# noirmist/Pytorch_Pose_Proposal_Network

Measured on AMD Instinct MI355X. Metric: images/sec (384x384, DRN-D-22) at 1/2/4/8 MI355X, higher is better.
Workload: dtype bf16

## Files before the change

pytorch_pose_proposal_network_amd/csrc/stem012.hip:

```cpp
#include <hip/hip_bf16.h>

#include <cstdlib>
#include <type_traits>
#include <utility>

#include "common.h"

#ifndef PPN_S012_SKIP
#define PPN_S012_SKIP 0
#endif


namespace {

typedef __attribute__((ext_vector_type(4))) float f32x4;
typedef __attribute__((ext_vector_type(8))) __bf16 bf16x8;
typedef __attribute__((ext_vector_type(8))) _Float16 f16x8;
typedef __attribute__((ext_vector_type(4))) __bf16 bf16x4;
typedef __attribute__((ext_vector_type(2))) unsigned u32x2;
typedef __attribute__((ext_vector_type(4))) unsigned u32x4;

constexpr int SW2 = 48;
constexpr int BAND2 = 16;
constexpr int NS = 7;
constexpr int W1 = NS * 16;
constexpr int W0 = W1 + 8;
#ifdef PPN_S012_OLD_L1
constexpr int W1P = W1;
#define PPN_S012_PQ(g) (g)
#define PPN_S012_LO(g) (2 * ((g) & 1))
constexpr int kHiPlanes = 1;
#else
constexpr int W1P = W1 + 1;
#define PPN_S012_PQ(g) ((((g) & 1) << 1) | ((g) >> 1))
#define PPN_S012_LO(g) ((g) & 1)
constexpr int kHiPlanes = 2;
#endif
constexpr int WI = W1 + 8;
constexpr int R0 = 6, R1 = 5, RI = 10;
constexpr int RAWS = 368;
constexpr int LDS_IN = RI * WI * 8, LDS_L0 = R0 * W0 * 32, LDS_L1 = R1 * 4 * W1P * 8, LDS_RAW = RI * RAWS, LDS_LUT = 3 * 256 * 2;
constexpr int LDS_CST = 4 * 32 * 4;
constexpr int LDS_BYTES = LDS_IN + LDS_L0 + LDS_L1 + LDS_RAW + LDS_LUT + LDS_CST;

struct Stem012Args {
    const void* src;
    const float *w0, *s0, *b0;
    const float *w1, *s1, *b1;
    const float *w2, *s2, *b2;
    const float *s3, *b3;
    void* out_raw;
    void* out_act;
    int B, H, W, Ho, Wo, src_is_u8;
    int raw_s2;
    float mean[3], stdv[3];
    int nstrips, nbands;
};

template <typename F, int... I>
__device__ __forceinline__ void sfor_impl(F&& f, std::integer_sequence<int, I...>) {
    (f(std::integral_constant<int, I>{}), ...);
}
template <int N, typename F>
__device__ __forceinline__ void sfor(F&& f) {
    sfor_impl(f, std::make_integer_sequence<int, N>{});
}

template <int OFF>
__device__ __forceinline__ u32x2 lds_read64(unsigned addr) {
    u32x2 v;
    asm volatile("ds_read_b64 %0, %1 offset:%2" : "=v"(v) : "v"(addr), "n"(OFF));
    return v;
}

__device__ __forceinline__ f32x4 mfma16(bf16x8 a, bf16x8 b, f32x4 c, int, int, int) { return __builtin_amdgcn_mfma_f32_16x16x32_bf16(a, b, c, 0, 0, 0); }
__device__ __forceinline__ f32x4 mfma16(f16x8 a, f16x8 b, f32x4 c, int, int, int) { return __builtin_amdgcn_mfma_f32_16x16x32_f16(a, b, c, 0, 0, 0); }

template <typename H>
__device__ __forceinline__ H to_store(float v) {
    if constexpr (sizeof(H) == 2 && !__is_same(H, __bf16)) return (H)fminf(v, 65504.f);
    else return (H)v;
}

template <typename H>
__device__ __forceinline__ u32x2 bn_relu_pack(const f32x4& acc, const float (&sc)[4], const float (&sh)[4], bool inside) {
    typedef __attribute__((ext_vector_type(4))) H hx4;
    hx4 o;
#pragma unroll
    for (int r = 0; r < 4; ++r) {
        const float t = acc[r] * sc[r] + sh[r];
        o[r] = to_store<H>(t > 0.f ? t : 0.f);
    }
    u32x2 p = __builtin_bit_cast(u32x2, o);
    p.x = inside ? p.x : 0u;
    p.y = inside ? p.y : 0u;
    return p;
}

template <bool U8, typename H, typename HO = H>
__global__ void __launch_bounds__(256, 2) stem012_kernel(Stem012Args a) {
    typedef __attribute__((ext_vector_type(8))) H hx8;
    typedef __attribute__((ext_vector_type(4))) H hx4;
    typedef __attribute__((ext_vector_type(4))) HO hox4;
    constexpr bool kExactIn = U8 && std::is_same<H, _Float16>::value;
    extern __shared__ __attribute__((aligned(16))) char smem[];
    char* in_p = smem;
    char* l0_p = smem + LDS_IN;
    char* l1_p = smem + LDS_IN + LDS_L0;
    char* raw_p = smem + LDS_IN + LDS_L0 + LDS_L1;
    unsigned short* lut_p = reinterpret_cast<unsigned short*>(smem + LDS_IN + LDS_L0 + LDS_L1 + LDS_RAW);
    const int tid = threadIdx.x, lane = tid & 63;
    const int wave = __builtin_amdgcn_readfirstlane(tid >> 6);
    const int ch = lane & 15, g = lane >> 4, col = lane & 15;

    hx8 wa0[7];
    hx8 wa1[5];
    hx8 wa2[2][5];
    {
        float* wl = reinterpret_cast<float*>(smem);
        constexpr int N0 = 16 * 147, N1 = 16 * 144, N2 = 32 * 144;
        static_assert((N0 + N1 + N2) * 4 <= LDS_IN + LDS_L0 + LDS_L1, "weight staging must fit below the raw rows / LUT");
        for (int i = tid; i < N0; i += 256) wl[i] = a.w0[i];
        for (int i = tid; i < N1; i += 256) wl[N0 + i] = a.w1[i];
        for (int i = tid; i < N2; i += 256) wl[N0 + N1 + i] = a.w2[i];
        __syncthreads();
        const float* wc = wl + ch * 3 * 49;
#pragma unroll
        for (int dy = 0; dy < 7; ++dy)
#pragma unroll
            for (int hf = 0; hf < 2; ++hf) {
                const int dx = 2 * g + hf;
                const bool ok = dx < 7;
                const int dxc = ok ? dx : 6;
                float w3[3];
#pragma unroll
                for (int c = 0; c < 3; ++c) w3[c] = wc[(c * 7 + dy) * 7 + dxc];
                if constexpr (kExactIn) {
                    float v = 0.f;
#pragma unroll
                    for (int c = 0; c < 3; ++c) {
                        wa0[dy][4 * hf + c] = (H)(ok ? w3[c] / a.stdv[c] : 0.f);
                        v += w3[c] * ((128.f - a.mean[c]) / a.stdv[c]);
                    }
                    wa0[dy][4 * hf + 3] = (H)(ok ? v : 0.f);
                } else {
#pragma unroll
                    for (int c = 0; c < 3; ++c) wa0[dy][4 * hf + c] = (H)(ok ? w3[c] : 0.f);
                    wa0[dy][4 * hf + 3] = (H)0.f;
                }
            }
        const float* wd = wl + N0 + ch * 16 * 9;
#pragma unroll
        for (int kk = 0; kk < 5; ++kk) {
            const int tap = 2 * kk + (g >> 1), tapc = tap < 9 ? tap : 8;
#pragma unroll
            for (int i = 0; i < 8; ++i) {
                const float v = wd[((g & 1) * 8 + i) * 9 + tapc];
                wa1[kk][i] = (H)(tap < 9 ? v : 0.f);
            }
        }
#pragma unroll
        for (int ct = 0; ct < 2; ++ct) {
            const float* we = wl + N0 + N1 + (ct * 16 + ch) * 16 * 9;
#pragma unroll
            for (int kk = 0; kk < 5; ++kk) {
                const int tap = 2 * kk + (g >> 1), tapc = tap < 9 ? tap : 8;
#pragma unroll
                for (int i = 0; i < 8; ++i) {
                    const float v = we[((g & 1) * 8 + i) * 9 + tapc];
                    wa2[ct][kk][i] = (H)(tap < 9 ? v : 0.f);
                }
            }
        }
    }
    float sc0[4], sh0[4], sc1[4], sh1[4];
#pragma unroll
    for (int r = 0; r < 4; ++r) {
        sc0[r] = a.s0[4 * g + r]; sh0[r] = a.b0[4 * g + r];
        sc1[r] = a.s1[4 * g + r]; sh1[r] = a.b1[4 * g + r];
    }
    float* cst_p = reinterpret_cast<float*>(smem + LDS_IN + LDS_L0 + LDS_L1 + LDS_RAW + LDS_LUT);
    if (tid < 128) {
        const int c = tid & 31, which = tid >> 5;
        float v;
        if (which == 0) v = a.s2[c];
        else if (which == 1) v = a.b2[c];
        else if (which == 2) v = a.s3 ? a.s3[c] : 1.f;
        else v = a.b3 ? a.b3[c] : 0.f;
        cst_p[tid] = v;
    }
    if constexpr (U8 && !kExactIn) {
        for (int i = tid; i < 3 * 256; i += 256) {
            const int c = i >> 8;
            const H v = (H)(((float)(i & 255) - a.mean[c]) / a.stdv[c]);
            lut_p[i] = __builtin_bit_cast(unsigned short, v);
        }
    }
    int tdy[5], tdx[5];
#pragma unroll
    for (int kk = 0; kk < 5; ++kk) {
        const int tap = 2 * kk + (g >> 1), t = tap < 9 ? tap : 0;
        tdy[kk] = t / 3; tdx[kk] = t - (t / 3) * 3;
    }
    const unsigned smem_base = (unsigned)(size_t)(__attribute__((address_space(3))) char*)smem;

    const int units = a.B * a.nbands * a.nstrips;
    for (int unit = blockIdx.x; unit < units; unit += gridDim.x) {
        int u = unit;
        const int strip = u % a.nstrips; u /= a.nstrips;
        const int band = u % a.nbands;
        const int b = u / a.nbands;
        const int C2 = strip * SW2, R2 = band * BAND2;
        const int R2e = min(R2 + BAND2, a.Ho);
        const int x0b = 2 * C2 - 2;
        const int x1b = 2 * C2 - 1;
        const int xib = 2 * C2 - 5;

        const int xs = xib < 0 ? 0 : xib;
        const int nb_row = (min(xib + WI, a.W) - xs) * 3;
        auto request_input = [&](int yi0, int nrows) {
            if constexpr (U8 && !(PPN_S012_SKIP & 16)) {
                const unsigned char* base = static_cast<const unsigned char*>(a.src);
                for (int q = wave; q < nrows * 2; q += 4) {
                    const int r = q >> 1, half = q & 1;
                    const int gy = yi0 + r;
                    if (gy < 0 || gy >= a.H) continue;
                    const size_t S = (((size_t)b * a.H + gy) * a.W + xs) * 3;
                    const size_t A = S & ~(size_t)3;
                    const int k = half * 64 + lane;
                    if (k < RAWS / 4 && A + 4 * (size_t)k < S + nb_row)
                        __builtin_amdgcn_global_load_lds((const void __attribute__((address_space(1)))*)(base + A + 4 * (size_t)k),
                                                         (void __attribute__((address_space(3)))*)(raw_p + r * RAWS + half * 256),
                                                         4, 0, 0);
                }
            }
        };
        auto convert_input = [&](int yi0, int nrows) {
            if (PPN_S012_SKIP & 1) return;
            if (tid >= 2 * WI) return;
            const int prow = tid >= WI ? 1 : 0, px = tid - prow * WI;
            const int gx = xib + px;
            const bool colok = gx >= 0 && gx < a.W;
            if constexpr (U8) {
                const unsigned base = smem_base + (unsigned)(LDS_IN + LDS_L0 + LDS_L1) + prow * RAWS + (colok ? (gx - xs) * 3 : 0);
                const unsigned sh0 = (((unsigned)b * a.H + (unsigned)(yi0 + prow)) * a.W + xs) * 3u;
                const unsigned dsh = 2u * a.W * 3u;
                unsigned v[RI / 2][3];
#pragma unroll
                for (int k = 0; k < RI / 2; ++k) {
                    const unsigned ad = base + 2 * k * RAWS + ((sh0 + k * dsh) & 3u);
                    asm volatile("ds_read_u8 %0, %1" : "=v"(v[k][0]) : "v"(ad));
                    asm volatile("ds_read_u8 %0, %1 offset:1" : "=v"(v[k][1]) : "v"(ad));
                    asm volatile("ds_read_u8 %0, %1 offset:2" : "=v"(v[k][2]) : "v"(ad));
                }
#define PPN_S012_WAIT15(v)                                                                                                   \
    asm volatile("s_waitcnt lgkmcnt(0)"                                                                                     \
                 : "+v"(v[0][0]), "+v"(v[0][1]), "+v"(v[0][2]), "+v"(v[1][0]), "+v"(v[1][1]), "+v"(v[1][2]), "+v"(v[2][0]),   \
                   "+v"(v[2][1]), "+v"(v[2][2]), "+v"(v[3][0]), "+v"(v[3][1]), "+v"(v[3][2]), "+v"(v[4][0]), "+v"(v[4][1]),   \
                   "+v"(v[4][2])::"memory")
                static_assert(RI / 2 == 5, "PPN_S012_WAIT15 names 5 x 3 values");
                PPN_S012_WAIT15(v);
                if constexpr (!kExactIn) {
                    const unsigned lb = smem_base + (unsigned)(LDS_IN + LDS_L0 + LDS_L1 + LDS_RAW);
#pragma unroll
                    for (int k = 0; k < RI / 2; ++k)
#pragma unroll
                        for (int c = 0; c < 3; ++c) {
                            const unsigned ad = lb + 512 * c + 2 * v[k][c];
                            asm volatile("ds_read_u16 %0, %1" : "=v"(v[k][c]) : "v"(ad));
                        }
                    PPN_S012_WAIT15(v);
                }
#pragma unroll
                for (int k = 0; k < RI / 2; ++k) {
                    const int py = prow + 2 * k;
                    if (py >= nrows) break;
                    const int gy = yi0 + py;
                    u32x2 o = {0u, 0u};
                    if (colok && gy >= 0 && gy < a.H) {
                        if constexpr (kExactIn) {
                            hx4 t;
#pragma unroll
                            for (int c = 0; c < 3; ++c) t[c] = (H)(float)((int)v[k][c] - 128);
                            t[3] = (H)1.f;
                            o = __builtin_bit_cast(u32x2, t);
                        } else {
                            o.x = v[k][0] | (v[k][1] << 16);
                            o.y = v[k][2];
                        }
                    }
                    *reinterpret_cast<u32x2*>(in_p + ((size_t)py * WI + px) * 8) = o;
                }
            } else {
#pragma unroll
                for (int k = 0; k < RI / 2; ++k) {
                    const int py = prow + 2 * k;
                    if (py >= nrows) break;
                    const int gy = yi0 + py;
                    u32x2 o = {0u, 0u};
                    if (colok && gy >= 0 && gy < a.H) {
                        const float* sp = static_cast<const float*>(a.src) + ((size_t)b * 3 * a.H + gy) * a.W + gx;
                        const size_t plane = (size_t)a.H * a.W;
                        hx4 t;
                        t[0] = (H)sp[0]; t[1] = (H)sp[plane]; t[2] = (H)sp[2 * plane]; t[3] = (H)0.f;
                        o = __builtin_bit_cast(u32x2, t);
                    }
                    *reinterpret_cast<u32x2*>(in_p + ((size_t)py * WI + px) * 8) = o;
                }
            }
        };
        auto input_landed = [&]() {
            asm volatile("s_waitcnt vmcnt(0) lgkmcnt(0)\n\ts_barrier" ::: "memory");
        };
        auto layer0 = [&](int y, int nrows) {
            if (PPN_S012_SKIP & 2) return;
            if (wave >= nrows) return;
            const int gy = y + wave;
            const bool rowok = gy >= 0 && gy < a.H;
            const unsigned rd = smem_base + (unsigned)((wave * WI + col + 2 * g) * 8);
            char* wr = l0_p + ((size_t)(((gy + 2 * R0) % R0) * 4 + g) * W0 + col) * 8;
            u32x2 lo[2][7], hi[2][7];
            auto fetch = [&](auto sgc, auto setc) {
                constexpr int sg = decltype(sgc)::value, st = decltype(setc)::value;
                sfor<7>([&](auto dyc) {
                    constexpr int dy = decltype(dyc)::value;
                    lo[st][dy] = lds_read64<dy * WI * 8 + sg * 128>(rd);
                    hi[st][dy] = lds_read64<dy * WI * 8 + sg * 128 + 8>(rd);
                });
            };
            fetch(std::integral_constant<int, 0>{}, std::integral_constant<int, 0>{});
            sfor<NS>([&](auto sgc) {
                constexpr int sg = decltype(sgc)::value, cur = sg & 1;
                if constexpr (sg + 1 < NS) {
                    fetch(std::integral_constant<int, sg + 1>{}, std::integral_constant<int, cur ^ 1>{});
                    asm volatile("s_waitcnt lgkmcnt(14)" ::: "memory");
                } else {
                    asm volatile("s_waitcnt lgkmcnt(0)" ::: "memory");
                }
                __builtin_amdgcn_sched_barrier(0);
                f32x4 acc = {0.f, 0.f, 0.f, 0.f};
#pragma unroll
                for (int dy = 0; dy < 7; ++dy) {
                    const u32x4 xb = {lo[cur][dy].x, lo[cur][dy].y, hi[cur][dy].x, hi[cur][dy].y};
                    acc = mfma16(wa0[dy], __builtin_bit_cast(hx8, xb), acc, 0, 0, 0);
                }
                const int gx = x0b + sg * 16 + col;
                *reinterpret_cast<u32x2*>(wr + sg * 128) = bn_relu_pack<H>(acc, sc0, sh0, rowok && gx >= 0 && gx < a.W);
            });
        };
        auto layer1 = [&](int y, int nrows) {
            if (PPN_S012_SKIP & 4) return;
            if (wave >= nrows) return;
            const int gy = y + wave;
            const bool rowok = gy >= 0 && gy < a.H;
            const int s0 = (gy - 1 + 2 * R0) % R0;
            unsigned rd[5];
#pragma unroll
            for (int kk = 0; kk < 5; ++kk) {
                int s = s0 + tdy[kk];
                s = s >= R0 ? s - R0 : s;
                rd[kk] = smem_base + (unsigned)(LDS_IN + ((s * 4 + 2 * (g & 1)) * W0 + col + tdx[kk]) * 8);
            }
            char* wr = l1_p + ((size_t)(((gy + 2 * R1) % R1) * 4 + PPN_S012_PQ(g)) * W1P + col) * 8;
            u32x2 lo[2][5], hi[2][5];
            auto fetch = [&](auto sgc, auto setc) {
                constexpr int sg = decltype(sgc)::value, st = decltype(setc)::value;
#pragma unroll
                for (int kk = 0; kk < 5; ++kk) {
                    lo[st][kk] = lds_read64<sg * 128>(rd[kk]);
                    hi[st][kk] = lds_read64<sg * 128 + W0 * 8>(rd[kk]);
#ifdef PPN_S012_DUP_L1
                    lo[st][kk] = lds_read64<sg * 128>(rd[kk]);
#endif
                }
            };
            fetch(std::integral_constant<int, 0>{}, std::integral_constant<int, 0>{});
            sfor<NS>([&](auto sgc) {
                constexpr int sg = decltype(sgc)::value, cur = sg & 1;
                if constexpr (sg + 1 < NS) {
                    fetch(std::integral_constant<int, sg + 1>{}, std::integral_constant<int, cur ^ 1>{});
#ifdef PPN_S012_DUP_L1
                    asm volatile("s_waitcnt lgkmcnt(15)" ::: "memory");
#else
                    asm volatile("s_waitcnt lgkmcnt(10)" ::: "memory");
#endif
                } else {
                    asm volatile("s_waitcnt lgkmcnt(0)" ::: "memory");
                }
                __builtin_amdgcn_sched_barrier(0);
                f32x4 acc = {0.f, 0.f, 0.f, 0.f};
#pragma unroll
                for (int kk = 0; kk < 5; ++kk) {
                    const u32x4 xb = {lo[cur][kk].x, lo[cur][kk].y, hi[cur][kk].x, hi[cur][kk].y};
                    acc = mfma16(wa1[kk], __builtin_bit_cast(hx8, xb), acc, 0, 0, 0);
                }
                const int gx = x1b + sg * 16 + col;
                *reinterpret_cast<u32x2*>(wr + sg * 128) = bn_relu_pack<H>(acc, sc1, sh1, rowok && gx >= 0 && gx < a.W);
            });
        };
        auto layer2 = [&](int oy0, int nrows) {
            if (PPN_S012_SKIP & 8) return;
            const int ry = wave >> 1;
            if (ry >= nrows) return;
            const int oy = oy0 + ry;
            const int s0 = (2 * oy - 1 + 2 * R1) % R1;
            const int sg0 = (wave & 1) * 2, nsg = (wave & 1) ? 1 : 2;
            unsigned rd[5];
#pragma unroll
            for (int kk = 0; kk < 5; ++kk) {
                int s = s0 + tdy[kk];
                s = s >= R1 ? s - R1 : s;
                rd[kk] = smem_base + (unsigned)(LDS_IN + LDS_L0 + ((s * 4 + PPN_S012_LO(g)) * W1P + 2 * (sg0 * 16 + col) + tdx[kk]) * 8);
            }
            for (int sg = 0; sg < nsg; ++sg) {
                const int ox = C2 + (sg0 + sg) * 16 + col;
                u32x2 lo[5], hi[5];
#pragma unroll
                for (int kk = 0; kk < 5; ++kk) {
                    lo[kk] = lds_read64<0>(rd[kk] + sg * 256);
                    hi[kk] = lds_read64<kHiPlanes * W1P * 8>(rd[kk] + sg * 256);
                }
                asm volatile("s_waitcnt lgkmcnt(0)" ::: "memory");
                __builtin_amdgcn_sched_barrier(0);
                f32x4 acc[2] = {{0.f, 0.f, 0.f, 0.f}, {0.f, 0.f, 0.f, 0.f}};
#pragma unroll
                for (int kk = 0; kk < 5; ++kk) {
                    const u32x4 xw = {lo[kk].x, lo[kk].y, hi[kk].x, hi[kk].y};
                    const hx8 xb = __builtin_bit_cast(hx8, xw);
#pragma unroll
                    for (int ct = 0; ct < 2; ++ct)
                        acc[ct] = mfma16(wa2[ct][kk], xb, acc[ct], 0, 0, 0);
                }
                if constexpr ((PPN_S012_SKIP & 32) != 0) {
                    asm volatile("" ::"v"(acc[0]), "v"(acc[1]));
                    continue;
                }
                if (oy < a.Ho && ox < a.Wo) {
                    const size_t pix = ((size_t)b * a.Ho + oy) * a.Wo + ox;
#pragma unroll
                    for (int ct = 0; ct < 2; ++ct) {
                        const f32x4 sc2 = *reinterpret_cast<const f32x4*>(cst_p + ct * 16 + 4 * g);
                        const f32x4 sh2 = *reinterpret_cast<const f32x4*>(cst_p + 32 + ct * 16 + 4 * g);
                        const f32x4 sc3 = *reinterpret_cast<const f32x4*>(cst_p + 64 + ct * 16 + 4 * g);
                        const f32x4 sh3 = *reinterpret_cast<const f32x4*>(cst_p + 96 + ct * 16 + 4 * g);
                        hox4 ov, ou;
#pragma unroll
                        for (int r = 0; r < 4; ++r) {
                            const float t = acc[ct][r] * sc2[r] + sh2[r];
                            const float v = t > 0.f ? t : 0.f;
                            const float w2 = v * sc3[r] + sh3[r];
                            ov[r] = to_store<HO>(v);
                            ou[r] = to_store<HO>(w2 > 0.f ? w2 : 0.f);
                        }
                        const size_t o = pix * 32 + ct * 16 + 4 * g;
                        if (a.out_raw) {
                            if (!a.raw_s2) *reinterpret_cast<hox4*>(static_cast<HO*>(a.out_raw) + o) = ov;
                            else if (((oy | ox) & 1) == 0)
                                *reinterpret_cast<hox4*>(static_cast<HO*>(a.out_raw) + ((((size_t)b * ((a.Ho + 1) >> 1) + (oy >> 1)) *
                                                         ((a.Wo + 1) >> 1) + (ox >> 1)) * 32 + ct * 16 + 4 * g)) = ov;
                        }
                        if (a.out_act) *reinterpret_cast<hox4*>(static_cast<HO*>(a.out_act) + o) = ou;
                    }
                }
            }
        };

        lds_barrier();
        request_input(2 * R2 - 5, 9);
        input_landed();
        convert_input(2 * R2 - 5, 9);
        lds_barrier();
        request_input(2 * R2 - 2, RI);
        layer0(2 * R2 - 2, 3);
        lds_barrier();
        layer1(2 * R2 - 1, 1);
        for (int r2 = R2; r2 < R2e; r2 += 2) {
            input_landed();
            convert_input(2 * r2 - 2, RI);
            lds_barrier();
            if (r2 + 2 < R2e) request_input(2 * r2 + 2, RI);
            if (r2 > R2) layer2(r2 - 2, 2);
            layer0(2 * r2 + 1, 4);
            lds_barrier();
            layer1(2 * r2, 4);
        }
        lds_barrier();
        const int last = R2 + ((R2e - R2 - 1) / 2) * 2;
        layer2(last, min(2, R2e - last));
    }
}

}

namespace ppn {
int stem012_x3_launch(int src_is_u8, const void* src, int batch, int h, int w, const float* w0, const float* s0,
                      const float* b0, const float* mean, const float* stdv, const float* w1, const float* s1,
                      const float* b1, const float* w2, const float* s2, const float* b2, const float* s3, const float* b3,
                      void* out_raw, void* out_act, hipStream_t st);

template <bool U8, typename H, typename HO = H>
static int stem012_launch_T(const Stem012Args& a, unsigned grid, hipStream_t st) {
    static int max_lds_set = 0;
    PPN_LDS_ONCE(max_lds_set, reinterpret_cast<const void*>(stem012_kernel<U8, H, HO>),
                 hipFuncAttributeMaxDynamicSharedMemorySize, LDS_BYTES);
    hipLaunchKernelGGL((stem012_kernel<U8, H, HO>), dim3(grid), dim3(256), LDS_BYTES, st, a);
    return PPN_OK;
}

int stem012_launch(int dtype, int src_is_u8, const void* src, int batch, int h, int w, const float* w0, const float* s0,
                   const float* b0, const float* mean, const float* stdv, const float* w1, const float* s1,
                   const float* b1, const float* w2, const float* s2, const float* b2, const float* s3, const float* b3,
                   void* out_raw, void* out_act, hipStream_t st) {
    if (!src || !w0 || !s0 || !b0 || !w1 || !s1 || !b1 || !w2 || !s2 || !b2 || (!out_raw && !out_act) || batch < 1 ||
        h < 1 || w < 1 || (s3 == nullptr) != (b3 == nullptr))
        return fail(PPN_E_INVALID, "ppn_stem012: bad arguments");
    if (src_is_u8 && (!mean || !stdv)) return fail(PPN_E_INVALID, "ppn_stem012: mean/std required for u8 input");
    if (dtype == PPN_STEM_IO(PPN_F16X3, PPN_F32))
        return stem012_x3_launch(src_is_u8, src, batch, h, w, w0, s0, b0, mean, stdv, w1, s1, b1, w2, s2, b2, s3, b3, out_raw,
                                 out_act, st);
    Stem012Args a;
    a.src = src; a.w0 = w0; a.s0 = s0; a.b0 = b0; a.w1 = w1; a.s1 = s1; a.b1 = b1; a.w2 = w2; a.s2 = s2; a.b2 = b2;
    a.s3 = s3; a.b3 = b3; a.out_raw = out_raw; a.out_act = out_act;
    a.B = batch; a.H = h; a.W = w; a.src_is_u8 = src_is_u8;
    a.Ho = (h + 2 - 3) / 2 + 1; a.Wo = (w + 2 - 3) / 2 + 1;
    for (int i = 0; i < 3; ++i) { a.mean[i] = mean ? mean[i] : 0.f; a.stdv[i] = stdv ? stdv[i] : 1.f; }
    a.nstrips = (a.Wo + SW2 - 1) / SW2; a.nbands = (a.Ho + BAND2 - 1) / BAND2;
    const long long units = (long long)batch * a.nstrips * a.nbands;
    if (units > 0x7fffffffLL) return fail(PPN_E_UNSUPPORTED, "too many tiles");
    if ((long long)batch * h * w * 3 > 0xffffffffLL) return fail(PPN_E_UNSUPPORTED, "frames too large for 32-bit byte offsets");
    static const int per_cu = getenv("PPN_S012_WGS") ? atoi(getenv("PPN_S012_WGS")) : 2;
    const unsigned grid = (unsigned)(units < 256 * per_cu ? units : 256 * per_cu);
    const int din = dtype & 0xff, dout = ((dtype >> 8) & 0xff) ? ((dtype >> 8) & 0xff) - 1 : din;
    a.raw_s2 = (dtype & PPN_STEM_RAW_S2) ? 1 : 0;
    if ((din != PPN_BF16 && din != PPN_F16) || (dout != PPN_BF16 && dout != PPN_F16) || (din == PPN_BF16 && dout != PPN_BF16))
        return fail(PPN_E_INVALID, "ppn_stem012: dtype must be PPN_BF16, PPN_F16, PPN_STEM_IO(PPN_F16, PPN_BF16) or "
                    "PPN_STEM_IO(PPN_F16X3, PPN_F32)");
    int rc;
    if (din == PPN_F16 && dout == PPN_BF16)
        rc = src_is_u8 ? stem012_launch_T<true, _Float16, __bf16>(a, grid, st) : stem012_launch_T<false, _Float16, __bf16>(a, grid, st);
    else if (din == PPN_F16)
        rc = src_is_u8 ? stem012_launch_T<true, _Float16>(a, grid, st) : stem012_launch_T<false, _Float16>(a, grid, st);
    else
        rc = src_is_u8 ? stem012_launch_T<true, __bf16>(a, grid, st) : stem012_launch_T<false, __bf16>(a, grid, st);
    if (rc != PPN_OK) return rc;
    PPN_LAUNCH_CHECK();
    return PPN_OK;
}
}

extern "C" int ppn_stem012(int32_t src_is_u8, const void* src, int32_t batch, int32_t h, int32_t w, const float* w0,
                           const float* scale0, const float* shift0, const float* mean, const float* std_,
                           const float* w1, const float* scale1, const float* shift1, const float* w2,
                           const float* scale2, const float* shift2, const float* scale3, const float* shift3,
                           void* out_raw, void* out_act, void* stream) {
    return ppn::stem012_launch(PPN_BF16, src_is_u8, src, batch, h, w, w0, scale0, shift0, mean, std_, w1, scale1, shift1,
                               w2, scale2, shift2, scale3, shift3, out_raw, out_act, static_cast<hipStream_t>(stream));
}

extern "C" int ppn_stem012_dt(int32_t dtype, int32_t src_is_u8, const void* src, int32_t batch, int32_t h, int32_t w,
                              const float* w0, const float* scale0, const float* shift0, const float* mean,
                              const float* std_, const float* w1, const float* scale1, const float* shift1,
                              const float* w2, const float* scale2, const float* shift2, const float* scale3,
                              const float* shift3, void* out_raw, void* out_act, void* stream) {
    return ppn::stem012_launch(dtype, src_is_u8, src, batch, h, w, w0, scale0, shift0, mean, std_, w1, scale1, shift1, w2,
                               scale2, shift2, scale3, shift3, out_raw, out_act, static_cast<hipStream_t>(stream));
}
```

Before: 11830.

## Turn stem input staging into a row ring and batch layer-0 rows per wave

Converts the input tile into a 12-row ring buffer so each band step fetches and converts only the 4 new raw rows instead of all 10. The warm-up rows borrow the layer-1 LDS region. Layer 0 is restructured so each wave computes 4 output rows for its column segments, reusing each loaded input row across several 7-tap MFMA accumulations. This reduces redundant global loads, u8 conversion and LDS reads. The cost is more accumulator registers, uneven work across waves (wave 3 gets one segment), and more intricate waitcnt and ring-index logic.

```diff
diff --git a/pytorch_pose_proposal_network_amd/csrc/stem012.hip b/pytorch_pose_proposal_network_amd/csrc/stem012.hip
--- a/pytorch_pose_proposal_network_amd/csrc/stem012.hip
+++ b/pytorch_pose_proposal_network_amd/csrc/stem012.hip
@@ -37,11 +37,15 @@
 constexpr int kHiPlanes = 2;
 #endif
 constexpr int WI = W1 + 8;
-constexpr int R0 = 6, R1 = 5, RI = 10;
+constexpr int R0 = 6, R1 = 5, RI = 12;
+constexpr int RNEW = 4, RWARM = 9;
 constexpr int RAWS = 368;
-constexpr int LDS_IN = RI * WI * 8, LDS_L0 = R0 * W0 * 32, LDS_L1 = R1 * 4 * W1P * 8, LDS_RAW = RI * RAWS, LDS_LUT = 3 * 256 * 2;
+constexpr int LDS_IN = RI * WI * 8, LDS_L0 = R0 * W0 * 32, LDS_L1 = R1 * 4 * W1P * 8, LDS_RAW = RNEW * RAWS, LDS_LUT = 3 * 256 * 2;
 constexpr int LDS_CST = 4 * 32 * 4;
 constexpr int LDS_BYTES = LDS_IN + LDS_L0 + LDS_L1 + LDS_RAW + LDS_LUT + LDS_CST;
+constexpr int OFF_L1 = LDS_IN + LDS_L0, OFF_RAW = OFF_L1 + LDS_L1;
+static_assert(RWARM * RAWS <= LDS_L1, "the warm-up's raw rows borrow the layer-1 ring");
+static_assert(RI % RNEW == 0 && RI >= RNEW + 6, "the ring holds the 4 + 6 rows a chunk's layer 0 reads, in whole chunks");
 
 struct Stem012Args {
     const void* src;
@@ -106,9 +110,8 @@
     extern __shared__ __attribute__((aligned(16))) char smem[];
     char* in_p = smem;
     char* l0_p = smem + LDS_IN;
-    char* l1_p = smem + LDS_IN + LDS_L0;
-    char* raw_p = smem + LDS_IN + LDS_L0 + LDS_L1;
-    unsigned short* lut_p = reinterpret_cast<unsigned short*>(smem + LDS_IN + LDS_L0 + LDS_L1 + LDS_RAW);
+    char* l1_p = smem + OFF_L1;
+    unsigned short* lut_p = reinterpret_cast<unsigned short*>(smem + OFF_RAW + LDS_RAW);
     const int tid = threadIdx.x, lane = tid & 63;
     const int wave = __builtin_amdgcn_readfirstlane(tid >> 6);
     const int ch = lane & 15, g = lane >> 4, col = lane & 15;
@@ -179,7 +182,7 @@
         sc0[r] = a.s0[4 * g + r]; sh0[r] = a.b0[4 * g + r];
         sc1[r] = a.s1[4 * g + r]; sh1[r] = a.b1[4 * g + r];
     }
-    float* cst_p = reinterpret_cast<float*>(smem + LDS_IN + LDS_L0 + LDS_L1 + LDS_RAW + LDS_LUT);
+    float* cst_p = reinterpret_cast<float*>(smem + OFF_RAW + LDS_RAW + LDS_LUT);
     if (tid < 128) {
         const int c = tid & 31, which = tid >> 5;
         float v;
@@ -218,134 +221,165 @@
 
         const int xs = xib < 0 ? 0 : xib;
         const int nb_row = (min(xib + WI, a.W) - xs) * 3;
-        auto request_input = [&](int yi0, int nrows) {
+        auto request_input = [&](int yi0, int nrows, int rawoff) {
             if constexpr (U8 && !(PPN_S012_SKIP & 16)) {
                 const unsigned char* base = static_cast<const unsigned char*>(a.src);
-                for (int q = wave; q < nrows * 2; q += 4) {
-                    const int r = q >> 1, half = q & 1;
+                char* raw_p = smem + rawoff;
+                for (int r = wave; r < nrows; r += 4) {
                     const int gy = yi0 + r;
                     if (gy < 0 || gy >= a.H) continue;
                     const size_t S = (((size_t)b * a.H + gy) * a.W + xs) * 3;
                     const size_t A = S & ~(size_t)3;
-                    const int k = half * 64 + lane;
-                    if (k < RAWS / 4 && A + 4 * (size_t)k < S + nb_row)
-                        __builtin_amdgcn_global_load_lds((const void __attribute__((address_space(1)))*)(base + A + 4 * (size_t)k),
-                                                         (void __attribute__((address_space(3)))*)(raw_p + r * RAWS + half * 256),
-                                                         4, 0, 0);
+#pragma unroll
+                    for (int half = 0; half < 2; ++half) {
+                        const int k = half * 64 + lane;
+                        if (k < RAWS / 4 && A + 4 * (size_t)k < S + nb_row)
+                            __builtin_amdgcn_global_load_lds((const void __attribute__((address_space(1)))*)(base + A + 4 * (size_t)k),
+                                                             (void __attribute__((address_space(3)))*)(raw_p + r * RAWS + half * 256),
+                                                             4, 0, 0);
+                    }
                 }
             }
         };
-        auto convert_input = [&](int yi0, int nrows) {
+        auto own_requests_landed = [&]() { asm volatile("s_waitcnt vmcnt(0)" ::: "memory"); };
+        auto convert_input = [&](auto npc, int yi0, int nrows, int slot0, int rawoff) {
+            constexpr int NP = decltype(npc)::value;
             if (PPN_S012_SKIP & 1) return;
-            if (tid >= 2 * WI) return;
-            const int prow = tid >= WI ? 1 : 0, px = tid - prow * WI;
-            const int gx = xib + px;
-            const bool colok = gx >= 0 && gx < a.W;
+            bool colok[2];
+#pragma unroll
+            for (int j = 0; j < 2; ++j) colok[j] = lane + 64 * j < WI && xib + lane + 64 * j >= 0 && xib + lane + 64 * j < a.W;
+            auto store = [&](int py, int j, u32x2 o) {
+                int sl = slot0 + py;
+                sl = sl >= RI ? sl - RI : sl;
+                if (lane + 64 * j < WI) *reinterpret_cast<u32x2*>(in_p + ((size_t)sl * WI + lane + 64 * j) * 8) = o;
+            };
             if constexpr (U8) {
-                const unsigned base = smem_base + (unsigned)(LDS_IN + LDS_L0 + LDS_L1) + prow * RAWS + (colok ? (gx - xs) * 3 : 0);
-                const unsigned sh0 = (((unsigned)b * a.H + (unsigned)(yi0 + prow)) * a.W + xs) * 3u;
-                const unsigned dsh = 2u * a.W * 3u;
-                unsigned v[RI / 2][3];
-#pragma unroll
-                for (int k = 0; k < RI / 2; ++k) {
-                    const unsigned ad = base + 2 * k * RAWS + ((sh0 + k * dsh) & 3u);
-                    asm volatile("ds_read_u8 %0, %1" : "=v"(v[k][0]) : "v"(ad));
-                    asm volatile("ds_read_u8 %0, %1 offset:1" : "=v"(v[k][1]) : "v"(ad));
-                    asm volatile("ds_read_u8 %0, %1 offset:2" : "=v"(v[k][2]) : "v"(ad));
-                }
-#define PPN_S012_WAIT15(v)                                                                                                   \
-    asm volatile("s_waitcnt lgkmcnt(0)"                                                                                     \
-                 : "+v"(v[0][0]), "+v"(v[0][1]), "+v"(v[0][2]), "+v"(v[1][0]), "+v"(v[1][1]), "+v"(v[1][2]), "+v"(v[2][0]),   \
-                   "+v"(v[2][1]), "+v"(v[2][2]), "+v"(v[3][0]), "+v"(v[3][1]), "+v"(v[3][2]), "+v"(v[4][0]), "+v"(v[4][1]),   \
-                   "+v"(v[4][2])::"memory")
-                static_assert(RI / 2 == 5, "PPN_S012_WAIT15 names 5 x 3 values");
-                PPN_S012_WAIT15(v);
+                unsigned v[NP][2][3];
+#pragma unroll
+                for (int k = 0; k < NP; ++k) {
+                    const int py = wave + 4 * k;
+                    const unsigned al = ((((unsigned)b * a.H + (unsigned)(yi0 + py)) * a.W + xs) * 3u) & 3u;
+#pragma unroll
+                    for (int j = 0; j < 2; ++j) {
+                        const unsigned ad = smem_base + (unsigned)rawoff + py * RAWS + (colok[j] ? (xib + lane + 64 * j - xs) * 3 : 0) + al;
+                        asm volatile("ds_read_u8 %0, %1" : "=v"(v[k][j][0]) : "v"(ad));
+                        asm volatile("ds_read_u8 %0, %1 offset:1" : "=v"(v[k][j][1]) : "v"(ad));
+                        asm volatile("ds_read_u8 %0, %1 offset:2" : "=v"(v[k][j][2]) : "v"(ad));
+                    }
+                }
+#define PPN_S012_TIE6(v, k) "+v"(v[k][0][0]), "+v"(v[k][0][1]), "+v"(v[k][0][2]), "+v"(v[k][1][0]), "+v"(v[k][1][1]), "+v"(v[k][1][2])
+#define PPN_S012_WAIT6(v) asm volatile("s_waitcnt lgkmcnt(0)" : PPN_S012_TIE6(v, 0)::"memory")
+#define PPN_S012_WAIT18(v) asm volatile("s_waitcnt lgkmcnt(0)" : PPN_S012_TIE6(v, 0), PPN_S012_TIE6(v, 1), PPN_S012_TIE6(v, 2)::"memory")
+                static_assert(NP == 1 || NP == 3, "PPN_S012_WAIT6 / PPN_S012_WAIT18 name 1 x 6 / 3 x 6 values");
+                static_assert((RNEW + 3) / 4 == 1 && (RWARM + 3) / 4 == 3, "rows per wave of a chunk / of the warm-up");
+                auto wait_all = [&]() {
+                    if constexpr (NP == 1) PPN_S012_WAIT6(v);
+                    else PPN_S012_WAIT18(v);
+                };
+                wait_all();
                 if constexpr (!kExactIn) {
-                    const unsigned lb = smem_base + (unsigned)(LDS_IN + LDS_L0 + LDS_L1 + LDS_RAW);
-#pragma unroll
-                    for (int k = 0; k < RI / 2; ++k)
-#pragma unroll
-                        for (int c = 0; c < 3; ++c) {
-                            const unsigned ad = lb + 512 * c + 2 * v[k][c];
-                            asm volatile("ds_read_u16 %0, %1" : "=v"(v[k][c]) : "v"(ad));
-                        }
-                    PPN_S012_WAIT15(v);
-                }
-#pragma unroll
-                for (int k = 0; k < RI / 2; ++k) {
-                    const int py = prow + 2 * k;
+                    const unsigned lb = smem_base + (unsigned)(OFF_RAW + LDS_RAW);
+#pragma unroll
+                    for (int k = 0; k < NP; ++k)
+#pragma unroll
+                        for (int j = 0; j < 2; ++j)
+#pragma unroll
+                            for (int c = 0; c < 3; ++c) {
+                                const unsigned ad = lb + 512 * c + 2 * v[k][j][c];
+                                asm volatile("ds_read_u16 %0, %1" : "=v"(v[k][j][c]) : "v"(ad));
+                            }
+                    wait_all();
+                }
+#pragma unroll
+                for (int k = 0; k < NP; ++k) {
+                    const int py = wave + 4 * k;
                     if (py >= nrows) break;
                     const int gy = yi0 + py;
-                    u32x2 o = {0u, 0u};
-                    if (colok && gy >= 0 && gy < a.H) {
-                        if constexpr (kExactIn) {
-                            hx4 t;
-#pragma unroll
-                            for (int c = 0; c < 3; ++c) t[c] = (H)(float)((int)v[k][c] - 128);
-                            t[3] = (H)1.f;
-                            o = __builtin_bit_cast(u32x2, t);
-                        } else {
-                            o.x = v[k][0] | (v[k][1] << 16);
-                            o.y = v[k][2];
+#pragma unroll
+                    for (int j = 0; j < 2; ++j) {
+                        u32x2 o = {0u, 0u};
+                        if (colok[j] && gy >= 0 && gy < a.H) {
+                            if constexpr (kExactIn) {
+                                hx4 t;
+#pragma unroll
+                                for (int c = 0; c < 3; ++c) t[c] = (H)(float)((int)v[k][j][c] - 128);
+                                t[3] = (H)1.f;
+                                o = __builtin_bit_cast(u32x2, t);
+                            } else {
+                                o.x = v[k][j][0] | (v[k][j][1] << 16);
+                                o.y = v[k][j][2];
+                            }
                         }
+                        store(py, j, o);
                     }
-                    *reinterpret_cast<u32x2*>(in_p + ((size_t)py * WI + px) * 8) = o;
                 }
             } else {
 #pragma unroll
-                for (int k = 0; k < RI / 2; ++k) {
-                    const int py = prow + 2 * k;
+                for (int k = 0; k < NP; ++k) {
+                    const int py = wave + 4 * k;
                     if (py >= nrows) break;
                     const int gy = yi0 + py;
-                    u32x2 o = {0u, 0u};
-                    if (colok && gy >= 0 && gy < a.H) {
-                        const float* sp = static_cast<const float*>(a.src) + ((size_t)b * 3 * a.H + gy) * a.W + gx;
-                        const size_t plane = (size_t)a.H * a.W;
-                        hx4 t;
-                        t[0] = (H)sp[0]; t[1] = (H)sp[plane]; t[2] = (H)sp[2 * plane]; t[3] = (H)0.f;
-                        o = __builtin_bit_cast(u32x2, t);
+#pragma unroll
+                    for (int j = 0; j < 2; ++j) {
+                        u32x2 o = {0u, 0u};
+                        if (colok[j] && gy >= 0 && gy < a.H) {
+                            const float* sp = static_cast<const float*>(a.src) + ((size_t)b * 3 * a.H + gy) * a.W + xib + lane + 64 * j;
+                            const size_t plane = (size_t)a.H * a.W;
+                            hx4 t;
+                            t[0] = (H)sp[0]; t[1] = (H)sp[plane]; t[2] = (H)sp[2 * plane]; t[3] = (H)0.f;
+                            o = __builtin_bit_cast(u32x2, t);
+                        }
+                        store(py, j, o);
                     }
-                    *reinterpret_cast<u32x2*>(in_p + ((size_t)py * WI + px) * 8) = o;
                 }
             }
         };
-        auto input_landed = [&]() {
-            asm volatile("s_waitcnt vmcnt(0) lgkmcnt(0)\n\ts_barrier" ::: "memory");
-        };
-        auto layer0 = [&](int y, int nrows) {
+        auto layer0 = [&](auto nrc, int y, int slot0) {
+            constexpr int NR = decltype(nrc)::value, NP = NR + 6;
+            static_assert(NP <= RI && NR <= RNEW, "a call reads NR + 6 distinct ring rows");
             if (PPN_S012_SKIP & 2) return;
-            if (wave >= nrows) return;
-            const int gy = y + wave;
-            const bool rowok = gy >= 0 && gy < a.H;
-            const unsigned rd = smem_base + (unsigned)((wave * WI + col + 2 * g) * 8);
-            char* wr = l0_p + ((size_t)(((gy + 2 * R0) % R0) * 4 + g) * W0 + col) * 8;
-            u32x2 lo[2][7], hi[2][7];
-            auto fetch = [&](auto sgc, auto setc) {
-                constexpr int sg = decltype(sgc)::value, st = decltype(setc)::value;
-                sfor<7>([&](auto dyc) {
-                    constexpr int dy = decltype(dyc)::value;
-                    lo[st][dy] = lds_read64<dy * WI * 8 + sg * 128>(rd);
-                    hi[st][dy] = lds_read64<dy * WI * 8 + sg * 128 + 8>(rd);
+            const int sgb = 2 * wave, nsg = wave == 3 ? 1 : 2;
+            unsigned rd[NP];
+#pragma unroll
+            for (int p = 0; p < NP; ++p) {
+                int s = slot0 + p;
+                s = s >= RI ? s - RI : s;
+                rd[p] = smem_base + (unsigned)((s * WI + sgb * 16 + col + 2 * g) * 8);
+            }
+            sfor<2>([&](auto ic) {
+                constexpr int i = decltype(ic)::value;
+                if (i >= nsg) return;
+                u32x2 lo[NP], hi[NP];
+                sfor<NP>([&](auto pc) {
+                    constexpr int p = decltype(pc)::value;
+                    lo[p] = lds_read64<i * 128>(rd[p]);
+                    hi[p] = lds_read64<i * 128 + 8>(rd[p]);
                 });
-            };
-            fetch(std::integral_constant<int, 0>{}, std::integral_constant<int, 0>{});
-            sfor<NS>([&](auto sgc) {
-                constexpr int sg = decltype(sgc)::value, cur = sg & 1;
-                if constexpr (sg + 1 < NS) {
-                    fetch(std::integral_constant<int, sg + 1>{}, std::integral_constant<int, cur ^ 1>{});
-                    asm volatile("s_waitcnt lgkmcnt(14)" ::: "memory");
-                } else {
-                    asm volatile("s_waitcnt lgkmcnt(0)" ::: "memory");
-                }
-                __builtin_amdgcn_sched_barrier(0);
-                f32x4 acc = {0.f, 0.f, 0.f, 0.f};
-#pragma unroll
-                for (int dy = 0; dy < 7; ++dy) {
-                    const u32x4 xb = {lo[cur][dy].x, lo[cur][dy].y, hi[cur][dy].x, hi[cur][dy].y};
-                    acc = mfma16(wa0[dy], __builtin_bit_cast(hx8, xb), acc, 0, 0, 0);
-                }
-                const int gx = x0b + sg * 16 + col;
-                *reinterpret_cast<u32x2*>(wr + sg * 128) = bn_relu_pack<H>(acc, sc0, sh0, rowok && gx >= 0 && gx < a.W);
+                f32x4 acc[NR];
+#pragma unroll
+                for (int r = 0; r < NR; ++r) acc[r] = f32x4{0.f, 0.f, 0.f, 0.f};
+                sfor<7>([&](auto dc) {
+                    constexpr int dy = decltype(dc)::value;
+                    sfor<(dy == 0 ? NR : 1)>([&](auto qc) {
+                        constexpr int p = dy == 0 ? decltype(qc)::value : dy + NR - 1;
+                        u32x2 &l = lo[p], &h = hi[p];
+                        asm volatile("s_waitcnt lgkmcnt(%2)" : "+v"(l), "+v"(h) : "n"(12 - 2 * dy) : "memory");
+                    });
+                    __builtin_amdgcn_sched_barrier(0);
+#pragma unroll
+                    for (int r = 0; r < NR; ++r) {
+                        const u32x4 xb = {lo[r + dy].x, lo[r + dy].y, hi[r + dy].x, hi[r + dy].y};
+                        acc[r] = mfma16(wa0[dy], __builtin_bit_cast(hx8, xb), acc[r], 0, 0, 0);
+                    }
+                });
+                const int gx = x0b + (sgb + i) * 16 + col;
+                const bool colok = gx >= 0 && gx < a.W;
+#pragma unroll
+                for (int r = 0; r < NR; ++r) {
+                    const int gy = y + r;
+                    *reinterpret_cast<u32x2*>(l0_p + ((size_t)(((gy + 2 * R0) % R0) * 4 + g) * W0 + (sgb + i) * 16 + col) * 8) =
+                        bn_relu_pack<H>(acc[r], sc0, sh0, colok && gy >= 0 && gy < a.H);
+                }
             });
         };
         auto layer1 = [&](int y, int nrows) {
@@ -466,23 +500,30 @@
         };
 
         lds_barrier();
-        request_input(2 * R2 - 5, 9);
-        input_landed();
-        convert_input(2 * R2 - 5, 9);
+        request_input(2 * R2 - 5, RWARM, OFF_L1);
+        own_requests_landed();
+        convert_input(std::integral_constant<int, (RWARM + 3) / 4>{}, 2 * R2 - 5, RWARM, 0, OFF_L1);
+        request_input(2 * R2 + 4, RNEW, OFF_RAW);
         lds_barrier();
-        request_input(2 * R2 - 2, RI);
-        layer0(2 * R2 - 2, 3);
+        layer0(std::integral_constant<int, 3>{}, 2 * R2 - 2, 0);
         lds_barrier();
         layer1(2 * R2 - 1, 1);
+        own_requests_landed();
+        convert_input(std::integral_constant<int, 1>{}, 2 * R2 + 4, RNEW, RWARM, OFF_RAW);
+        int ph = RWARM;
         for (int r2 = R2; r2 < R2e; r2 += 2) {
-            input_landed();
-            convert_input(2 * r2 - 2, RI);
+            const int phn = ph + RNEW >= RI ? ph + RNEW - RI : ph + RNEW;
             lds_barrier();
-            if (r2 + 2 < R2e) request_input(2 * r2 + 2, RI);
+            if (r2 + 2 < R2e) request_input(2 * r2 + 8, RNEW, OFF_RAW);
             if (r2 > R2) layer2(r2 - 2, 2);
-            layer0(2 * r2 + 1, 4);
+            layer0(std::integral_constant<int, 4>{}, 2 * r2 + 1, ph >= 6 ? ph - 6 : ph + 6);
             lds_barrier();
             layer1(2 * r2, 4);
+            if (r2 + 2 < R2e) {
+                own_requests_landed();
+                convert_input(std::integral_constant<int, 1>{}, 2 * r2 + 8, RNEW, phn, OFF_RAW);
+            }
+            ph = phn;
         }
         lds_barrier();
         const int last = R2 + ((R2e - R2 - 1) / 2) * 2;
```

Result: no change. 11840, median of 3 (+0.1%).
